# CatOfTheCannals/MPI_blockchain

Measured on AMD Instinct MI355X. Metric: SHA-256 nonce trials/sec (whole job) + % int32 VALU peak, higher is better.
Workload: dtype u32

## Files before the change

mpi_blockchain_amd/csrc/pow_api.cpp:

```cpp
#include <sys/prctl.h>

#include <algorithm>
#include <chrono>
#include <cstdio>
#include <cstring>
#include <ctime>
#include <thread>
#include <vector>

#include "pow_ctx.h"

#ifndef POW_WAIT_POLL_US
#define POW_WAIT_POLL_US 50
#endif

const pow_test_hooks* pow_hooks = nullptr;

namespace {

int stage_result(pow_ctx* ctx, bool with_tail, uint64_t abs_start);

void fill_watch(const pow_ctx* ctx, PowWatch& w, uint64_t abs_start) {
  memset(&w, 0, sizeof w);
  w.watch_epoch = ctx->watch_epoch && ctx->armed.load(std::memory_order_acquire) ? 1u : 0u;
  w.host_epoch = ctx->d_epoch;
  w.launch_epoch = ctx->launch_epoch;
  w.abs_start = abs_start;
  if (ctx->board && !ctx->board_off) {
    w.board = ctx->board_dev;
    w.board_mine = const_cast<unsigned long long*>(ctx->board_dev) + ctx->board_slot;
    w.board_n = (uint32_t)pow_board_nslots(ctx->board);
    w.board_tag = ctx->board_tag;
  }
}

uint64_t board_peer_min(const pow_ctx* ctx) {
  uint64_t m = UINT64_MAX;
  if (ctx->board && !ctx->board_off) pow_board_peek(ctx->board, ctx->board_slot, ctx->board_tag, &m);
  return m;
}

int set_dev(const pow_ctx* ctx) {
  HIP_OK(hipSetDevice(ctx->device));
  return POW_OK;
}

int stream_wait(pow_ctx* ctx, const char* what, uint64_t t0, uint64_t deadline_ns, bool nap) {
  HIP_OK(hipEventRecord(ctx->ev_block, ctx->stream));
  const int slack = nap ? prctl(PR_GET_TIMERSLACK, 0, 0, 0, 0) : 0;
  if (slack > 1000) prctl(PR_SET_TIMERSLACK, 1000ul, 0, 0, 0);
  hipError_t q;
  bool late = false;
  for (uint32_t n = 1; (q = hipEventQuery(ctx->ev_block)) == hipErrorNotReady; ++n) {
    if (nap) std::this_thread::sleep_for(std::chrono::microseconds(POW_WAIT_POLL_US));
    if ((nap || (n & 255u) == 0) && mono_ns() > deadline_ns) {
      late = true;
      break;
    }
  }
  if (slack > 1000) prctl(PR_SET_TIMERSLACK, (unsigned long)slack, 0, 0, 0);
  if (late) {
    ctx->wedged = true;
    return fail(POW_EHIP, "%s: watchdog: not complete after %.3f s (deadline %.3f s; hipStreamQuery: %s); "
                "the context must not be reused",
                what, (mono_ns() - t0) * 1e-9, (deadline_ns - t0) * 1e-9, hipGetErrorString(hipStreamQuery(ctx->stream)));
  }
  HIP_OK(q);
  HIP_OK(hipStreamSynchronize(ctx->stream));
  return POW_OK;
}

int stream_wait_for(pow_ctx* ctx, const char* what, uint64_t extra_ns) {
  const uint64_t t0 = mono_ns();
  return stream_wait(ctx, what, t0, t0 + ctx->watchdog_ns + extra_ns, false);
}

unsigned grid_for(const pow_ctx* ctx, uint32_t n_prefix) {
  const uint64_t want = ((uint64_t)n_prefix + 255) / 256;
  return (unsigned)std::max<uint64_t>(1, std::min<uint64_t>(want, ctx->grid_full));
}

int run_search(pow_ctx* ctx, uint64_t start, uint64_t count, unsigned diff, uint32_t mode,
               uint32_t* dev_out, uint32_t cap) {
  PowLaunch L;
  int rc = make_launch(start, count, diff, cap, mode, &L);
  if (rc) return rc;
  if (ctx->sentinel_idle && mode >= 1) L.mode |= POW_LAUNCH_SENTINEL_IDLE;
  if (int rc2 = stage_result(ctx, true, start)) return rc2;
  const unsigned grid = grid_for(ctx, L.n_prefix);
  if (pow_hooks)
    if (int rc2 = pow_hooks->before_launch(ctx)) return rc2;
  HIP_OK(hipEventRecord(ctx->ev0, ctx->stream));
  HIP_OK(pow_launch_search((int)mode, diff > 32 || ctx->force_full, grid, ctx->stream, ctx->d_consts, L, dev_out,
                           ctx->d_res));
  HIP_OK(hipEventRecord(ctx->ev1, ctx->stream));
  HIP_OK(hipMemcpyAsync(ctx->h_res, ctx->d_res, sizeof(PowResult), hipMemcpyDeviceToHost, ctx->stream));
  {
    char what[160];
    snprintf(what, sizeof what, "search kernel (mode %u, %llu counters from %llu, d = %u)", mode,
             (unsigned long long)count, (unsigned long long)start, diff);
    const uint64_t t0 = mono_ns();
    if (int rc2 = stream_wait(ctx, what, t0, t0 + ctx->watchdog_ns + 2ull * count, count >= (1ull << 26)))
      return rc2;
  }
  float ms = 0;
  HIP_OK(hipEventElapsedTime(&ms, ctx->ev0, ctx->ev1));
  ctx->stats.kernel_ms += ms;
  ctx->stats.launches += 1;
  ctx->stats.hashes += mode >= 1 ? ctx->h_res->hashes : (uint64_t)L.n_prefix * POW_J;
  return POW_OK;
}

int wait_published(pow_ctx* ctx, const volatile uint32_t* done, const volatile uint32_t* started, uint32_t seq,
                   const char* what, uint64_t t0, uint64_t deadline_ns) {
  for (uint32_t n = 1; __atomic_load_n(const_cast<const uint32_t*>(done), __ATOMIC_ACQUIRE) != seq; ++n) {
    if ((n & 0xFFFFu) != 0) continue;
    int st;
    hipError_t q = hipSuccess;
    if (ctx->aql) {
      st = pow_hooks->path_status(ctx);
    } else {
      q = hipStreamQuery(ctx->stream);
      st = q == hipErrorNotReady ? 1 : q == hipSuccess ? 0 : -1;
    }
    if (st == 1) {
      if (mono_ns() <= deadline_ns) continue;
      const uint32_t seen = __atomic_load_n(const_cast<const uint32_t*>(done), __ATOMIC_ACQUIRE);
      if (seen == seq) break;
      std::string path = "launch path hip, hipStreamQuery: not ready";
      if (ctx->aql) path = pow_hooks->path_diag(ctx);
      const uint32_t st_word = __atomic_load_n(const_cast<const uint32_t*>(started), __ATOMIC_ACQUIRE);
      ctx->wedged = true;
      return fail(POW_EHIP,
                  "%s: watchdog: no result after %.3f s (seq %u, done word %u; the kernel %s (started word %u); %s); "
                  "the context must not be reused",
                  what, (mono_ns() - t0) * 1e-9, seq, seen,
                  st_word == seq ? "started: its first workgroup ran" : "never started", st_word, path.c_str());
    }
    if (__atomic_load_n(const_cast<const uint32_t*>(done), __ATOMIC_ACQUIRE) == seq) break;
    if (st < 0 && ctx->aql) return fail(POW_EHIP, "%s: the dispatch queue reported HSA status 0x%x", what, -st);
    HIP_OK(q);
    return fail(POW_EHIP, "%s ended without publishing its result (seq %u, done word %u)", what, seq,
                __atomic_load_n(const_cast<const uint32_t*>(done), __ATOMIC_ACQUIRE));
  }
  return POW_OK;
}

}

int launch_hash_one(pow_ctx* ctx, const PowMsg& M, uint32_t seq, uint64_t deadline_ns) {
  if (pow_hooks) {
    if (int sent = pow_hooks->dispatch_hash_one(ctx, M, seq, deadline_ns)) return sent < 0 ? sent : POW_OK;
    if (int rc = pow_hooks->before_launch(ctx)) return rc;
  }
  HIP_OK(pow_launch_hash_one(ctx->stream, M, ctx->d_one, seq));
  return POW_OK;
}

int launch_search_lat(pow_ctx* ctx, bool full, bool any, bool asm_groups, unsigned grid, const PowLaunchLat& L,
                      uint64_t deadline_ns) {
  if (pow_hooks) {
    if (int sent = pow_hooks->dispatch_lat(ctx, full, any, asm_groups, grid, L, deadline_ns))
      return sent < 0 ? sent : POW_OK;
// ... 22 lines not shown
  if (int rc = wait_published(ctx, &ctx->h_lat->done, &ctx->h_lat->started, L.seq, "latency kernel", t0, deadline))
    return rc;
  memcpy(ctx->h_res, (const void*)ctx->h_lat, sizeof(PowResult));
  const double ms = (double)ctx->h_res->ticks / ctx->realtime_khz;
  ctx->stats.kernel_ms += ms;
  ctx->stats.launches += 1;
  ctx->stats.hashes += ctx->h_res->hashes;
  return POW_OK;
}

int upload_consts(pow_ctx* ctx, const pow_block* tmpl) {
  pow_build_consts(tmpl, &ctx->h_blob->consts);
  const PowConsts& C = ctx->h_blob->consts;
  PowConstsLat& Q = ctx->lat_consts;
  memcpy(Q.kw, C.kw, sizeof Q.kw);
  memcpy(Q.st0, C.st0, sizeof Q.st0);
  memcpy(Q.kw0, C.kw0, sizeof Q.kw0);
  memcpy(Q.k, C.k, sizeof Q.k);
  memcpy(Q.w0raw, C.w0raw, sizeof Q.w0raw);
  ctx->consts_dirty = true;
  return POW_OK;
}

int stage_result(pow_ctx* ctx, bool with_tail, uint64_t abs_start) {
  PowResult& r = ctx->h_blob->res;
  memset(&r, 0, sizeof r);
  r.min_rel = ~0ull;
  r.peer_abs = ~0ull;
  fill_watch(ctx, r.watch, abs_start);
  if (with_tail) {
    r.tail_buf = ctx->d_tail;
    r.tail_cap = ctx->tail_cap;
  }
  const size_t off = ctx->consts_dirty ? 0 : offsetof(PowBlob, res);
  HIP_OK(hipMemcpyAsync((char*)ctx->d_blob + off, (const char*)ctx->h_blob + off, sizeof(PowBlob) - off,
                        hipMemcpyHostToDevice, ctx->stream));
  ctx->consts_dirty = false;
  return POW_OK;
}

}

bool cancel_moved(const volatile uint32_t* cancel_word, uint32_t epoch) {
  return cancel_word && __atomic_load_n(const_cast<const uint32_t*>(cancel_word), __ATOMIC_ACQUIRE) != epoch;
}

int pow_ctx_device(const pow_ctx* ctx) { return ctx->device; }
bool pow_ctx_wedged(const pow_ctx* ctx) { return ctx->wedged; }
void pow_ctx_set_stats(pow_ctx* ctx, const pow_stats& s) { ctx->stats = s; }
void* pow_ctx_stream(const pow_ctx* ctx) { return (void*)ctx->stream; }
int pow_ctx_stream_wait(pow_ctx* ctx, const char* what, uint64_t budget_ns) {
  return stream_wait_for(ctx, what, budget_ns);
}

extern "C" {

int pow_device_count(int* n) {
  if (!n) return fail(POW_EINVAL, "null");
  *n = 0;
  HIP_OK(hipGetDeviceCount(n));
// ... 17 lines not shown
  ctx->cu_count = prop.multiProcessorCount;
  {
    int rt = 0;
    if (hipDeviceGetAttribute(&rt, hipDeviceAttributeWallClockRate, device) == hipSuccess && rt > 0)
      ctx->realtime_khz = rt;
  }
  ctx->clock_khz = prop.clockRate;
  snprintf(ctx->name, sizeof ctx->name, "%s", prop.name);
  ctx->grid_full = (unsigned)prop.multiProcessorCount * 8u - 1u;
  if (pow_hooks) pow_hooks->configure(ctx);
  int rc = POW_OK;
  auto chk = [&](hipError_t e, const char* what) {
    if (e != hipSuccess && rc == POW_OK) rc = fail(POW_EHIP, "%s: %s", what, hipGetErrorString(e));
  };
  chk(hipStreamCreateWithFlags(&ctx->stream, hipStreamNonBlocking), "hipStreamCreate");
  chk(hipEventCreate(&ctx->ev0), "hipEventCreate");
  chk(hipEventCreate(&ctx->ev1), "hipEventCreate");
  chk(hipEventCreateWithFlags(&ctx->ev_block, hipEventDisableTiming), "hipEventCreate");
  chk(hipMalloc(&ctx->d_blob, sizeof(PowBlob)), "hipMalloc consts/result");
  if (ctx->d_blob) chk(hipMemsetAsync(ctx->d_blob, 0, sizeof(PowBlob), ctx->stream), "hipMemsetAsync");
  chk(hipMalloc(&ctx->d_lat, sizeof(PowResult)), "hipMalloc latency result");
  chk(hipHostMalloc(&ctx->h_lat, sizeof(PowResult), hipHostMallocMapped | hipHostMallocCoherent),
      "hipHostMalloc latency result");
  if (ctx->d_lat && ctx->h_lat) {
    PowResult* init = ctx->h_lat;
    memset(init, 0, sizeof *init);
    init->min_rel = ~0ull;
    init->peer_abs = ~0ull;
    chk(hipMemcpyAsync(ctx->d_lat, init, sizeof *init, hipMemcpyHostToDevice, ctx->stream), "hipMemcpyAsync");
    if (rc == POW_OK) rc = stream_wait_for(ctx, "pow_init copies", 0);
    chk(hipHostGetDevicePointer((void**)&ctx->d_lat_host, ctx->h_lat, 0), "hipHostGetDevicePointer");
  }
  chk(hipHostMalloc(&ctx->h_one, sizeof(PowHashOut), hipHostMallocMapped | hipHostMallocCoherent),
      "hipHostMalloc hash result");
  if (ctx->h_one) {
    memset(ctx->h_one, 0, sizeof(PowHashOut));
    chk(hipHostGetDevicePointer((void**)&ctx->d_one, ctx->h_one, 0), "hipHostGetDevicePointer");
  }
  chk(hipHostMalloc(&ctx->h_epoch, 64, hipHostMallocMapped | hipHostMallocCoherent), "hipHostMalloc epoch");
  if (ctx->h_epoch) {
    *ctx->h_epoch = 0;
    chk(hipHostGetDevicePointer((void**)&ctx->d_epoch, ctx->h_epoch, 0), "hipHostGetDevicePointer");
  }
  chk(hipHostMalloc(&ctx->h_blob, sizeof(PowBlob), hipHostMallocDefault), "hipHostMalloc staging");
  if (ctx->d_blob) {
    ctx->d_consts = &ctx->d_blob->consts;
    ctx->d_res = &ctx->d_blob->res;
  }
  chk(hipHostMalloc(&ctx->h_res, sizeof(PowResult), hipHostMallocDefault), "hipHostMalloc");
  ctx->tail_cap = ctx->grid_full * 4u * 32u;
  chk(hipMalloc(&ctx->d_tail, (size_t)ctx->tail_cap * sizeof(uint32_t)), "hipMalloc sweep tail");
  if (rc == POW_OK && pow_hooks) pow_hooks->open_path(ctx);
// ... 32 lines not shown
  if (ctx->h_brec) (void)hipHostFree(ctx->h_brec);
  (void)hipFree(ctx->d_race);
  (void)hipFree(ctx->d_rin);
  (void)hipFree(ctx->d_rslot);
  if (ctx->h_race) (void)hipHostFree(ctx->h_race);
  if (ctx->h_rin) (void)hipHostFree(ctx->h_rin);
  if (ctx->h_res) (void)hipHostFree(ctx->h_res);
  if (ctx->ev0) (void)hipEventDestroy(ctx->ev0);
  if (ctx->ev1) (void)hipEventDestroy(ctx->ev1);
  if (ctx->ev_block) (void)hipEventDestroy(ctx->ev_block);
  if (ctx->stream) (void)hipStreamDestroy(ctx->stream);
  if (ctx->h_epoch) (void)hipHostFree(ctx->h_epoch);
  (void)hipFree(ctx->d_lat);
  if (ctx->h_lat) (void)hipHostFree(ctx->h_lat);
  if (ctx->h_one) (void)hipHostFree(ctx->h_one);
  delete ctx;
}

int pow_warmup(pow_ctx* ctx) {
  if (!ctx) return fail(POW_EINVAL, "null");
  if (int rc = set_dev(ctx)) return rc;
  PowLaunch L;
  memset(&L, 0, sizeof L);
  PowLaunchLat LL;
  memset(&LL, 0, sizeof LL);
  LL.nwg = 1;
  for (int mode = 0; mode < 3; ++mode)
    for (int full = 0; full < 2; ++full)
      HIP_OK(pow_launch_search(mode, full != 0, 1, ctx->stream, ctx->d_consts, L, nullptr, ctx->d_res));
  for (int any = 0; any < 2; ++any)
    for (int full = 0; full < 2; ++full)
      for (int grp = 0; grp < 2; ++grp)
        HIP_OK(pow_launch_search_lat(full != 0, any != 0, grp != 0, 1, ctx->stream, ctx->lat_consts, LL,
                                     ctx->d_lat, ctx->d_lat_host));
  HIP_OK(pow_launch_hash(0, ctx->stream, nullptr, nullptr));
  PowMsg M;
  memset(&M, 0, sizeof M);
  HIP_OK(pow_launch_hash_one(ctx->stream, M, ctx->d_one, 0));
  if (int rc = stream_wait_for(ctx, "warm-up launches", 0)) return rc;
  if (pow_hooks)
    if (int rc = pow_hooks->warm_path(ctx, LL, M)) return rc;
  pow_block b;
  memset(&b, 0, sizeof b);
  return pow_hash_blocks(ctx, &b, 1, nullptr, nullptr);
}

// ... 225 lines not shown
  uint64_t step = use_lat ? std::max<uint64_t>(1ull << 12, 1ull << (dcap + 4))
                          : (any ? 1ull << 30 : std::max<uint64_t>(1ull << 12, 1ull << std::min(dcap + 2, 30u)));
  auto preempted = [&](uint64_t next) {
    const uint64_t m = board_peer_min(ctx);
    return any ? m != UINT64_MAX : m < next;
  };
  uint64_t done = 0;
  bool first = true;
  while (done < ctr_count) {
    if (cancel_moved(cancel_word, epoch) || preempted(ctr_start + done)) break;
    const bool lat = first && use_lat;
    const uint64_t cap = lat ? ctx->lat_max : (uint64_t)1 << 30;
    const uint64_t n = std::min<uint64_t>(std::min<uint64_t>(step, cap), ctr_count - done);
    const uint64_t s0 = ctr_start + done;
    if (int rc = lat ? run_search_lat(ctx, s0, n, diff_bits, any, lat_wps)
                     : run_search(ctx, s0, n, diff_bits, any ? 2 : 1, nullptr, 0))
      return rc;
    first = false;
    done += n;
    if (cancel_moved(cancel_word, epoch) || ctx->h_res->cancelled) break;
    if (ctx->h_res->min_rel != ~0ull) {
      const PowResult& r = *ctx->h_res;
      const PowHit* h = nullptr;
      for (uint32_t k = 0; lat && k < std::min<uint32_t>(r.nhit, POW_HITS); ++k) {
        const PowHit* c = &r.hit[k];
        if (any ? (!h || c->rel < h->rel) : c->rel == r.min_rel) h = c;
      }
      const uint64_t ctr = s0 + (h ? h->rel : r.min_rel);
      if (!any && board_peer_min(ctx) < ctr) break;
      *out = *tmpl;
      pow_nonce_from_counter(ctr, out->nonce);
      char hx[65];
      if (h) {
        digest_out(h->digest, nullptr, hx);
      } else {
        const pow_stats keep = ctx->stats;
        ctx->watch_epoch = false;
        ctx->board_off = true;
        const int rc = run_search_lat(ctx, ctr, 1, 0, true, 1);
        ctx->board_off = false;
        if (rc) return rc;
        ctx->stats = keep;
        const PowResult& w = *ctx->h_res;
        if (w.nhit < 1 || w.hit[0].rel != 0) return fail(POW_EHIP, "winner re-hash recorded no digest");
        digest_out(w.hit[0].digest, nullptr, hx);
      }
      memcpy(out->block_hash, hx, 65);
// ... 504 lines not shown
```

mpi_blockchain_amd/csrc/pow_kernels.hip:

```cpp
#include <hip/hip_runtime.h>
#include <stdint.h>

#include "pow_template.h"
#include "sha256_dev.h"

using namespace powdev;


namespace {

__device__ __forceinline__ uint32_t digit_char(uint32_t d) {
  return d + (d < 26u ? 97u : (d < 52u ? 39u : 0xFFFFFFFCu));
}

__device__ __forceinline__ unsigned long long uniform64(unsigned long long v) {
  uint32_t lo = __builtin_amdgcn_readfirstlane((uint32_t)v);
  uint32_t hi = __builtin_amdgcn_readfirstlane((uint32_t)(v >> 32));
  return ((unsigned long long)hi << 32) | lo;
}

typedef const __attribute__((address_space(4))) uint32_t* cptr;

__device__ __forceinline__ cptr as_const(const uint32_t* p) {
  return (cptr)(const __attribute__((address_space(1))) uint32_t*)p;
}

__device__ __forceinline__ cptr pin(cptr p, uint32_t dep) {
  asm volatile("" : "+s"(p) : "v"(dep));
  return p;
}

template <bool ASM>
__device__ __forceinline__ void const_chunk_lds(St& t, const uint32_t* lkw) {
  if (ASM) {
    POW_SB();
    const uint4 v0 = *reinterpret_cast<const uint4*>(lkw);
    POW_SB();
    t = rounds4_asm_from(t, v0.x, v0.y, v0.z, v0.w);
#pragma unroll
    for (int g = 4; g < 64; g += 4) {
      POW_SB();
      const uint4 v = *reinterpret_cast<const uint4*>(lkw + g);
      POW_SB();
      rounds4_asm(t, v.x, v.y, v.z, v.w);
    }
    POW_SB();
  } else {
#pragma unroll
    for (int g = 0; g < 64; g += 4) {
      const uint4 v = *reinterpret_cast<const uint4*>(lkw + g);
      round_kw_o(t, v.x);
      round_kw_o(t, v.y);
// ... 52 lines not shown
  const uint32_t n = nst & ~31u;
  unsigned long long got = 0;
  if (lane == 0) got = atomicAdd(&res->count, (unsigned long long)n);
  const unsigned long long base = uniform64(got);
  const uint32_t i = lane * 4u;
  if (i < n) {
    const uint32_t e0 = wst[i], e1 = wst[i + 1u], e2 = wst[i + 2u], e3 = wst[i + 3u];
    const unsigned long long o = base + i;
    if (o + 4u <= cap && ((uintptr_t)out & 15u) == 0) {
      *reinterpret_cast<uint4*>(out + o) = make_uint4(e0, e1, e2, e3);
    } else {
      if (o < cap) out[o] = e0;
      if (o + 1u < cap) out[o + 1u] = e1;
      if (o + 2u < cap) out[o + 2u] = e2;
      if (o + 3u < cap) out[o + 3u] = e3;
    }
  }
  const uint32_t rem = nst - n;
  const uint32_t t = lane < rem ? wst[n + lane] : 0u;
  if (lane < rem) wst[lane] = t;
  nst = rem;
}

__device__ __forceinline__ void flush_tail(const uint32_t* wst, uint32_t nst, uint32_t lane, PowResult* res) {
  uint32_t got = 0;
  if (lane == 0) got = atomicAdd(&res->tail, nst);
  const uint32_t base = __builtin_amdgcn_readfirstlane(got);
  uint32_t* const tail = res->tail_buf;
  const uint32_t tail_cap = res->tail_cap;
  if (lane < nst && base + lane < tail_cap) tail[base + lane] = wst[lane];
}

__device__ __forceinline__ bool poll_stop(const PowWatch& w, unsigned int* cancelled, unsigned long long* peer_abs,
                                          unsigned long long lowest_abs) {
  const uint32_t watch = w.watch_epoch;
  const unsigned long long* const board = w.board;
  if (!watch && !board) return false;
  if (blockIdx.x == 0 && threadIdx.x < 64u) {
    const uint32_t lane = threadIdx.x;
    if (watch) {
      const unsigned int now = __hip_atomic_load(w.host_epoch, __ATOMIC_RELAXED, __HIP_MEMORY_SCOPE_SYSTEM);
      if ((uint32_t)__builtin_amdgcn_readfirstlane(now) != w.launch_epoch && lane == 0)
        __hip_atomic_store(cancelled, 1u, __ATOMIC_RELAXED, __HIP_MEMORY_SCOPE_AGENT);
    }
    if (board) {
      unsigned long long c = ~0ull;
      if (lane < w.board_n && board + lane != w.board_mine) {
        const unsigned long long v = __hip_atomic_load(board + lane, __ATOMIC_RELAXED, __HIP_MEMORY_SCOPE_SYSTEM);
        if ((uint32_t)(v >> POW_BOARD_SHIFT) == w.board_tag && (v & POW_BOARD_NONE) != POW_BOARD_NONE)
          c = v & POW_BOARD_NONE;
      }
#pragma unroll
// ... 15 lines not shown
  if (mine)
    __hip_atomic_store(mine, ((unsigned long long)w.board_tag << POW_BOARD_SHIFT) | (w.abs_start + rel),
                       __ATOMIC_RELAXED, __HIP_MEMORY_SCOPE_SYSTEM);
}

__device__ __forceinline__ bool full_test(const uint32_t H[8], uint32_t d) { return leading_zero_bits(H) >= d; }

}

#define POW_BATCH 8u

template <int MODE, bool FULL>
__global__ __launch_bounds__(256) __attribute__((amdgpu_num_sgpr(80), amdgpu_waves_per_eu(8))) void pow_search(
    const PowConsts* __restrict__ C, PowLaunch L, uint32_t* __restrict__ out,
    PowResult* __restrict__ res) {
  const uint32_t lane = threadIdx.x & 63u;
  uint32_t iters = 0;
  __shared__ __attribute__((aligned(16))) uint32_t stage[4][256];
  uint32_t* wst = stage[threadIdx.x >> 6];
  uint32_t nst = 0;
  uint32_t mymin = 0xFFFFFFFFu;
  __shared__ __attribute__((aligned(16))) uint32_t lkw[4 * 64];
  lkw[threadIdx.x] = (&C->kw[0][0])[threadIdx.x];
  __shared__ uint32_t sibs_done;
  __shared__ uint32_t wg_tick;
  __shared__ unsigned long long wg_ring[4];
  __shared__ uint32_t wg_reads[4];
  if (threadIdx.x == 0) {
    sibs_done = 0;
    wg_tick = 0;
  }
  if (threadIdx.x < 4) {
    wg_ring[threadIdx.x] = 0;
    wg_reads[threadIdx.x] = POW_BATCH - 1u;
  }
  __syncthreads();

  const bool sentinel_idle = MODE >= 1 && (L.mode & POW_LAUNCH_SENTINEL_IDLE) && blockIdx.x == 0 && threadIdx.x < 64u;
  for (;;) {
    if (sentinel_idle) break;
    uint32_t got = 0;
    if (lane == 0) {
      const uint32_t t = atomicAdd(&wg_tick, 1u);
      const uint32_t b = t / POW_BATCH, slot = t % POW_BATCH;
      unsigned long long* const ring = &wg_ring[b & 3u];
      uint32_t* const reads = &wg_reads[b & 3u];
      if (slot == 0) {
        got = atomicAdd(&res->next, 64u * POW_BATCH);
        while (__hip_atomic_load(reads, __ATOMIC_ACQUIRE, __HIP_MEMORY_SCOPE_WORKGROUP) != POW_BATCH - 1u)
          __builtin_amdgcn_s_sleep(1);
        __hip_atomic_store(reads, 0u, __ATOMIC_RELAXED, __HIP_MEMORY_SCOPE_WORKGROUP);
        __hip_atomic_store(ring, ((unsigned long long)(b + 1u) << 32) | got, __ATOMIC_RELEASE,
                           __HIP_MEMORY_SCOPE_WORKGROUP);
      } else {
        unsigned long long v;
        while ((uint32_t)((v = __hip_atomic_load(ring, __ATOMIC_ACQUIRE, __HIP_MEMORY_SCOPE_WORKGROUP)) >> 32) !=
               b + 1u)
          __builtin_amdgcn_s_sleep(1);
        got = (uint32_t)v + 64u * slot;
        __hip_atomic_fetch_add(reads, 1u, __ATOMIC_RELEASE, __HIP_MEMORY_SCOPE_WORKGROUP);
      }
    }
    const uint32_t rbase = __builtin_amdgcn_readfirstlane(got);
    if (rbase >= L.n_prefix) break;
    if (MODE >= 1) {
      unsigned long long f =
          __hip_atomic_load(&res->min_rel, __ATOMIC_RELAXED, __HIP_MEMORY_SCOPE_AGENT);
      f = uniform64(f);
      long long lo = (long long)rbase * 62 - (long long)L.off0;
      if (MODE == 2 && f != ~0ull) break;
      if (lo > 0 && f < (unsigned long long)lo) break;
      if (poll_stop(res->watch, &res->cancelled, &res->peer_abs,
                    MODE == 2 ? ~0ull : res->watch.abs_start + (lo > 0 ? (unsigned long long)lo : 0ull)))
        break;
    }
    const uint32_t r = rbase + lane;

    uint32_t dg[8];
    {
      uint32_t x = r, carry = 0;
#pragma unroll
      for (int i = 7; i >= 0; --i) {
        uint32_t q = x / 62u;
        uint32_t s = L.base_digit[i] + (x - q * 62u) + carry;
        x = q;
        carry = s >= 62u ? 1u : 0u;
        dg[i] = carry ? s - 62u : s;
      }
    }
    const uint32_t W1 = (digit_char(dg[0]) << 24) | (digit_char(dg[1]) << 16) |
                        (digit_char(dg[2]) << 8) | digit_char(dg[3]);
    const uint32_t W2 = (digit_char(dg[4]) << 24) | (digit_char(dg[5]) << 16) |
                        (digit_char(dg[6]) << 8) | digit_char(dg[7]);

    St s2{C->st0[0], C->st0[1], C->st0[2], C->st0[3], C->st0[4], C->st0[5], C->st0[6], C->st0[7]};
    round_k_w(s2, K[1], W1);
    round_k_w(s2, K[2], W2);
    const uint32_t W16 = C->u16 + ssig0(W1);
    const uint32_t W17 = C->u17 + ssig0(W2) + W1;
    const uint32_t c18 = ssig1(W16) + W2;
    const uint32_t c19 = ssig1(W17) + C->u19;
    const uint32_t c23 = W16 + C->u23;
    const uint32_t c24 = W17 + C->u24;
    const uint32_t c31 = ssig0(W16) + C->w15;
    const uint32_t c32 = ssig0(W17) + W16;
    const uint32_t P3 = s2.h + bsig1(s2.e) + ch(s2.e, s2.f, s2.g);
    const uint32_t A3 = P3 + bsig0(s2.a) + maj(s2.a, s2.b, s2.c);
    const uint32_t E3 = s2.d + P3;

    bool stop = false;
    for (uint32_t j = 0; j < POW_J; ++j) {
      if (MODE == 1 && j != 0 && (j & 1u) == 0) {
        unsigned long long f =
            __hip_atomic_load(&res->min_rel, __ATOMIC_RELAXED, __HIP_MEMORY_SCOPE_AGENT);
        f = uniform64(f);
        long long lo = (long long)rbase * 62 + j - (long long)L.off0;
        if (lo > 0 && f < (unsigned long long)lo) break;
        if (poll_stop(res->watch, &res->cancelled, &res->peer_abs,
                      res->watch.abs_start + (lo > 0 ? (unsigned long long)lo : 0ull))) {
          stop = true;
          break;
        }
      }
      if (MODE == 2 && j != 0) {
        unsigned long long f =
            __hip_atomic_load(&res->min_rel, __ATOMIC_RELAXED, __HIP_MEMORY_SCOPE_AGENT);
        if (uniform64(f) != ~0ull || poll_stop(res->watch, &res->cancelled, &res->peer_abs, ~0ull)) {
          stop = true;
          break;
        }
      }
      ++iters;
      cptr Cb = as_const(reinterpret_cast<const uint32_t*>(C));
      cptr J = pin(Cb, s2.a ^ j);
      const uint32_t kw3 = J[PC_KW3 + j];
      const St s4{A3 + kw3, s2.a, s2.b, s2.c, E3 + kw3, s2.e, s2.f, s2.g};
      asm volatile(".p2align 3");
      POW_SB();
      St s = rounds4_kws_asm_from(s4, J[PC_KW0 + 4], J[PC_KW0 + 5], J[PC_KW0 + 6], J[PC_KW0 + 7]);
#pragma unroll
      for (int i = 8; i < 16; i += 4) {
        POW_SB();
        rounds4_kws_asm(s, J[PC_KW0 + i], J[PC_KW0 + i + 1], J[PC_KW0 + i + 2], J[PC_KW0 + i + 3]);
      }
      uint32_t w[64];
      w[16] = W16;
      w[17] = W17;
      auto rnd4 = [&](int i, cptr Kx) {
        if (i >= 36) {
          POW_SB();
// ... 32 lines not shown
        cptr K3 = pin(Cb + PC_K, s.e);
#pragma unroll
        for (int i = 48; i < 64; i += 4) rnd4(i, K3);
      }
      uint32_t H[8] = {IV[0] + s.a, IV[1] + s.b, IV[2] + s.c, IV[3] + s.d,
                       IV[4] + s.e, IV[5] + s.f, IV[6] + s.g, IV[7] + s.h};

      St Hs{H[0], H[1], H[2], H[3], H[4], H[5], H[6], H[7]};
      St t = Hs;
      const_chunk_lds<true>(t, lkw);
#pragma unroll
      for (int c = 1; c < 4; ++c) const_chunk_lds_ff(Hs, t, lkw + 64 * c);
      const uint32_t h0 = Hs.a + t.a;

      bool hit = h0 <= L.thr;
      if (FULL && hit) {
        uint32_t D[8] = {h0, Hs.b + t.b, Hs.c + t.c, Hs.d + t.d,
                         Hs.e + t.e, Hs.f + t.f, Hs.g + t.g, Hs.h + t.h};
        hit = full_test(D, L.diff);
      }
      if (MODE != 0) {
        if (__builtin_expect(hit, 0)) {
          const unsigned long long rel = (unsigned long long)r * 62ull + j - L.off0;
          if (rel < L.count && rel < atomicMin(&res->min_rel, rel)) publish_hit(res->watch, rel);
        }
      } else {
        bool ok = false;
        uint32_t relv = 0;
        if (__builtin_expect(hit, 0)) {
          const unsigned long long rel = (unsigned long long)r * 62ull + j - L.off0;
          ok = rel < L.count;
          relv = (uint32_t)rel;
          if (ok && relv < mymin) mymin = relv;
          if (ok && relv == 0xFFFFFFFFu) atomicMin(&res->min_rel, rel);
        }
        const unsigned long long m = __ballot(ok);
        if (m) {
          const uint32_t rank = __builtin_amdgcn_mbcnt_hi((uint32_t)(m >> 32),
                                                          __builtin_amdgcn_mbcnt_lo((uint32_t)m, 0u));
          if (ok) wst[nst + rank] = relv;
          nst += (uint32_t)__popcll(m);
          if (nst >= 192) flush_stage(wst, nst, lane, res, out, L.cap);
        }
      }
    }
    if (MODE >= 1 && stop) break;
  }
  if (MODE == 0) {
    if (nst >= 32) flush_stage(wst, nst, lane, res, out, L.cap);
    if (nst) flush_tail(wst, nst, lane, res);
#pragma unroll
    for (int off = 32; off > 0; off >>= 1) {
      const uint32_t o = __shfl_xor(mymin, off, 64);
      mymin = o < mymin ? o : mymin;
    }
    if (lane == 0 && mymin != 0xFFFFFFFFu) atomicMin(&res->min_rel, (unsigned long long)mymin);
  }
  if (MODE >= 1) {
    if (blockIdx.x == 0) {
      if (threadIdx.x >= 64u) {
        if (lane == 0) __hip_atomic_fetch_add(&sibs_done, 1u, __ATOMIC_RELAXED, __HIP_MEMORY_SCOPE_WORKGROUP);
      } else if (res->watch.watch_epoch || res->watch.board) {
        for (;;) {
          const uint32_t sd = __hip_atomic_load(&sibs_done, __ATOMIC_RELAXED, __HIP_MEMORY_SCOPE_WORKGROUP);
          const uint32_t ex = __hip_atomic_load(&res->wg_exits, __ATOMIC_RELAXED, __HIP_MEMORY_SCOPE_AGENT);
          if (__builtin_amdgcn_readfirstlane(sd) >= (blockDim.x >> 6) - 1u &&
              __builtin_amdgcn_readfirstlane(ex) >= gridDim.x - 1u)
            break;
          (void)poll_stop(res->watch, &res->cancelled, &res->peer_abs, ~0ull);
          __builtin_amdgcn_s_sleep(32);
        }
      }
    }
    __shared__ uint32_t wave_iters[4];
    if ((threadIdx.x & 63u) == 0) wave_iters[threadIdx.x >> 6] = iters;
    __syncthreads();
    if (threadIdx.x == 0) {
      atomicAdd(&res->hashes,
                (unsigned long long)(wave_iters[0] + wave_iters[1] + wave_iters[2] + wave_iters[3]) * 64ull);
      if (blockIdx.x != 0) atomicAdd(&res->wg_exits, 1u);
    }
  }
}

template __global__ void pow_search<0, false>(const PowConsts*, PowLaunch, uint32_t*, PowResult*);
template __global__ void pow_search<0, true>(const PowConsts*, PowLaunch, uint32_t*, PowResult*);
template __global__ void pow_search<1, false>(const PowConsts*, PowLaunch, uint32_t*, PowResult*);
template __global__ void pow_search<1, true>(const PowConsts*, PowLaunch, uint32_t*, PowResult*);
template __global__ void pow_search<2, false>(const PowConsts*, PowLaunch, uint32_t*, PowResult*);
template __global__ void pow_search<2, true>(const PowConsts*, PowLaunch, uint32_t*, PowResult*);

template <bool FULL, bool ANY, bool ASM>
__global__ __launch_bounds__(256) void pow_search_lat(
    const PowConstsLat C0, PowLaunchLat L, PowResult* __restrict__ res, PowResult* __restrict__ hout) {
  (void)C0;
  const cptr Cb = (cptr)__builtin_amdgcn_kernarg_segment_ptr();
  const uint32_t lane = threadIdx.x & 63u;
  const uint32_t wave = __builtin_amdgcn_readfirstlane(blockIdx.x * 4u + (threadIdx.x >> 6));
  const uint32_t nwaves = L.nwg * 4u;
  uint32_t iters = 0;
  bool wrote_hit = false;
  __shared__ uint32_t wg_iters;
  if (threadIdx.x == 0) wg_iters = 0;
// ... 232 lines not shown
```

mpi_blockchain_amd/csrc/pow_template.h:

```cpp
#pragma once
#include <stdint.h>

#define POW_J 62

struct PowConsts {
  uint32_t kw[4][64];
  uint32_t st0[8];
  uint32_t kw0[16];
  uint32_t w0, w1_unused, w2_unused, w3lo;
  uint32_t u16;
  uint32_t u17;
  uint32_t u19;
  uint32_t u20, u21, u22;
  uint32_t u23, u24;
  uint32_t u25[6];
  uint32_t w15;
  uint32_t pad[3];
  uint32_t kw3[POW_J];
  uint32_t u18[POW_J];
  uint32_t w3[POW_J];
  uint32_t k[64];
  uint32_t w0raw[16];
};

// ... 24 lines not shown

struct PowWatch {
  const unsigned int* host_epoch;
  const unsigned long long* board;
  unsigned long long* board_mine;
  unsigned long long abs_start;
  uint32_t watch_epoch;
  uint32_t launch_epoch;
  uint32_t board_n;
  uint32_t board_tag;
};

struct PowLaunchLat {
  uint32_t base_digit[9];
  uint32_t thr;
  uint32_t diff;
  uint32_t seq;
  uint64_t count;
  PowWatch watch;
  uint32_t nwg;
  uint32_t pad;
};

struct PowLaunch {
  uint32_t base_digit[8];
  uint32_t n_prefix;
  uint32_t off0;
  uint64_t count;
  uint32_t thr;
  uint32_t diff;
  uint32_t cap;
  uint32_t mode;
};
#define POW_LAUNCH_SENTINEL_IDLE 0x100u

#define POW_HITS 8
struct PowHit {
  unsigned long long rel;
  uint32_t digest[8];
};

struct PowResult {
  unsigned long long min_rel;
  unsigned long long hashes;
  unsigned long long count;
  unsigned int next;
  unsigned int wg_exits;
  unsigned int tail;
  unsigned int tail_cap;
  unsigned int* tail_buf;
  unsigned int nhit;
  unsigned int cancelled;
  unsigned long long peer_abs;
  PowWatch watch;
  unsigned long long t_start;
  unsigned long long ticks;
  unsigned int done;
  unsigned int started;
  PowHit hit[POW_HITS];
};

struct PowMsg {
  uint32_t kw[5][64];
};
struct PowHashOut {
  uint32_t digest[8];
  unsigned long long ticks;
  unsigned int done;
  unsigned int started;
};

struct PowBlob {
  PowConsts consts;
  alignas(256) PowResult res;
};

#ifdef __cplusplus
// ... 19 lines not shown
```

Baseline: 9.138 billion.

## Publish search results via mapped host memory and self-reset device state in kernel

Per-launch watch and tail parameters now travel in kernel arguments, so the host-to-device copy that staged the result struct before every launch is gone. The last workgroup to finish resets the device result struct and writes the summary, hits and a done sequence word into mapped coherent host memory. The host polls that word instead of recording events and issuing a device-to-host copy. Kernel time is taken from device realtime ticks except in mode 0. This adds last-block election logic, more kernel-argument reads in the hot loop and extra atomics on hits, and correctness now depends on the in-kernel reset.

```diff
diff --git a/mpi_blockchain_amd/csrc/pow_api.cpp b/mpi_blockchain_amd/csrc/pow_api.cpp
--- a/mpi_blockchain_amd/csrc/pow_api.cpp
+++ b/mpi_blockchain_amd/csrc/pow_api.cpp
@@ -17,8 +17,6 @@
 const pow_test_hooks* pow_hooks = nullptr;
 
 namespace {
-
-int stage_result(pow_ctx* ctx, bool with_tail, uint64_t abs_start);
 
 void fill_watch(const pow_ctx* ctx, PowWatch& w, uint64_t abs_start) {
   memset(&w, 0, sizeof w);
@@ -45,20 +43,16 @@
   return POW_OK;
 }
 
-int stream_wait(pow_ctx* ctx, const char* what, uint64_t t0, uint64_t deadline_ns, bool nap) {
+int stream_wait(pow_ctx* ctx, const char* what, uint64_t t0, uint64_t deadline_ns) {
   HIP_OK(hipEventRecord(ctx->ev_block, ctx->stream));
-  const int slack = nap ? prctl(PR_GET_TIMERSLACK, 0, 0, 0, 0) : 0;
-  if (slack > 1000) prctl(PR_SET_TIMERSLACK, 1000ul, 0, 0, 0);
   hipError_t q;
   bool late = false;
   for (uint32_t n = 1; (q = hipEventQuery(ctx->ev_block)) == hipErrorNotReady; ++n) {
-    if (nap) std::this_thread::sleep_for(std::chrono::microseconds(POW_WAIT_POLL_US));
-    if ((nap || (n & 255u) == 0) && mono_ns() > deadline_ns) {
+    if ((n & 255u) == 0 && mono_ns() > deadline_ns) {
       late = true;
       break;
     }
   }
-  if (slack > 1000) prctl(PR_SET_TIMERSLACK, (unsigned long)slack, 0, 0, 0);
   if (late) {
     ctx->wedged = true;
     return fail(POW_EHIP, "%s: watchdog: not complete after %.3f s (deadline %.3f s; hipStreamQuery: %s); "
@@ -72,7 +66,7 @@
 
 int stream_wait_for(pow_ctx* ctx, const char* what, uint64_t extra_ns) {
   const uint64_t t0 = mono_ns();
-  return stream_wait(ctx, what, t0, t0 + ctx->watchdog_ns + extra_ns, false);
+  return stream_wait(ctx, what, t0, t0 + ctx->watchdog_ns + extra_ns);
 }
 
 unsigned grid_for(const pow_ctx* ctx, uint32_t n_prefix) {
@@ -80,44 +74,34 @@
   return (unsigned)std::max<uint64_t>(1, std::min<uint64_t>(want, ctx->grid_full));
 }
 
-int run_search(pow_ctx* ctx, uint64_t start, uint64_t count, unsigned diff, uint32_t mode,
-               uint32_t* dev_out, uint32_t cap) {
-  PowLaunch L;
-  int rc = make_launch(start, count, diff, cap, mode, &L);
-  if (rc) return rc;
-  if (ctx->sentinel_idle && mode >= 1) L.mode |= POW_LAUNCH_SENTINEL_IDLE;
-  if (int rc2 = stage_result(ctx, true, start)) return rc2;
-  const unsigned grid = grid_for(ctx, L.n_prefix);
-  if (pow_hooks)
-    if (int rc2 = pow_hooks->before_launch(ctx)) return rc2;
-  HIP_OK(hipEventRecord(ctx->ev0, ctx->stream));
-  HIP_OK(pow_launch_search((int)mode, diff > 32 || ctx->force_full, grid, ctx->stream, ctx->d_consts, L, dev_out,
-                           ctx->d_res));
-  HIP_OK(hipEventRecord(ctx->ev1, ctx->stream));
-  HIP_OK(hipMemcpyAsync(ctx->h_res, ctx->d_res, sizeof(PowResult), hipMemcpyDeviceToHost, ctx->stream));
-  {
-    char what[160];
-    snprintf(what, sizeof what, "search kernel (mode %u, %llu counters from %llu, d = %u)", mode,
-             (unsigned long long)count, (unsigned long long)start, diff);
-    const uint64_t t0 = mono_ns();
-    if (int rc2 = stream_wait(ctx, what, t0, t0 + ctx->watchdog_ns + 2ull * count, count >= (1ull << 26)))
-      return rc2;
-  }
-  float ms = 0;
-  HIP_OK(hipEventElapsedTime(&ms, ctx->ev0, ctx->ev1));
-  ctx->stats.kernel_ms += ms;
-  ctx->stats.launches += 1;
-  ctx->stats.hashes += mode >= 1 ? ctx->h_res->hashes : (uint64_t)L.n_prefix * POW_J;
-  return POW_OK;
-}
-
 int wait_published(pow_ctx* ctx, const volatile uint32_t* done, const volatile uint32_t* started, uint32_t seq,
-                   const char* what, uint64_t t0, uint64_t deadline_ns) {
+                   const char* what, uint64_t t0, uint64_t deadline_ns, uint64_t nap_from_ns = UINT64_MAX,
+                   const char* late = "watchdog: no result after", bool on_stream = false) {
+  const bool direct = ctx->aql && !on_stream;
+  struct Slack {
+    int was = 0;
+    void lower() {
+      if (was) return;
+      was = prctl(PR_GET_TIMERSLACK, 0, 0, 0, 0);
+      if (was > 1000) prctl(PR_SET_TIMERSLACK, 1000ul, 0, 0, 0);
+    }
+    ~Slack() {
+      if (was > 1000) prctl(PR_SET_TIMERSLACK, (unsigned long)was, 0, 0, 0);
+    }
+  } slack;
+  bool nap = nap_from_ns == 0;
   for (uint32_t n = 1; __atomic_load_n(const_cast<const uint32_t*>(done), __ATOMIC_ACQUIRE) != seq; ++n) {
-    if ((n & 0xFFFFu) != 0) continue;
+    if (nap) {
+      slack.lower();
+      std::this_thread::sleep_for(std::chrono::microseconds(POW_WAIT_POLL_US));
+      if ((n & 15u) != 0) continue;
+    } else {
+      if (nap_from_ns != UINT64_MAX && (n & 0xFFu) == 0 && mono_ns() >= nap_from_ns) nap = true;
+      if ((n & 0xFFFFu) != 0) continue;
+    }
     int st;
     hipError_t q = hipSuccess;
-    if (ctx->aql) {
+    if (direct) {
       st = pow_hooks->path_status(ctx);
     } else {
       q = hipStreamQuery(ctx->stream);
@@ -128,17 +112,17 @@
       const uint32_t seen = __atomic_load_n(const_cast<const uint32_t*>(done), __ATOMIC_ACQUIRE);
       if (seen == seq) break;
       std::string path = "launch path hip, hipStreamQuery: not ready";
-      if (ctx->aql) path = pow_hooks->path_diag(ctx);
+      if (direct) path = pow_hooks->path_diag(ctx);
       const uint32_t st_word = __atomic_load_n(const_cast<const uint32_t*>(started), __ATOMIC_ACQUIRE);
       ctx->wedged = true;
       return fail(POW_EHIP,
-                  "%s: watchdog: no result after %.3f s (seq %u, done word %u; the kernel %s (started word %u); %s); "
+                  "%s: %s %.3f s (seq %u, done word %u; the kernel %s (started word %u); %s); "
                   "the context must not be reused",
-                  what, (mono_ns() - t0) * 1e-9, seq, seen,
+                  what, late, (mono_ns() - t0) * 1e-9, seq, seen,
                   st_word == seq ? "started: its first workgroup ran" : "never started", st_word, path.c_str());
     }
     if (__atomic_load_n(const_cast<const uint32_t*>(done), __ATOMIC_ACQUIRE) == seq) break;
-    if (st < 0 && ctx->aql) return fail(POW_EHIP, "%s: the dispatch queue reported HSA status 0x%x", what, -st);
+    if (st < 0 && direct) return fail(POW_EHIP, "%s: the dispatch queue reported HSA status 0x%x", what, -st);
     HIP_OK(q);
     return fail(POW_EHIP, "%s ended without publishing its result (seq %u, done word %u)", what, seq,
                 __atomic_load_n(const_cast<const uint32_t*>(done), __ATOMIC_ACQUIRE));
@@ -207,20 +191,50 @@
   return POW_OK;
 }
 
-int stage_result(pow_ctx* ctx, bool with_tail, uint64_t abs_start) {
-  PowResult& r = ctx->h_blob->res;
-  memset(&r, 0, sizeof r);
-  r.min_rel = ~0ull;
-  r.peer_abs = ~0ull;
-  fill_watch(ctx, r.watch, abs_start);
-  if (with_tail) {
-    r.tail_buf = ctx->d_tail;
-    r.tail_cap = ctx->tail_cap;
-  }
-  const size_t off = ctx->consts_dirty ? 0 : offsetof(PowBlob, res);
-  HIP_OK(hipMemcpyAsync((char*)ctx->d_blob + off, (const char*)ctx->h_blob + off, sizeof(PowBlob) - off,
-                        hipMemcpyHostToDevice, ctx->stream));
-  ctx->consts_dirty = false;
+int run_search(pow_ctx* ctx, uint64_t start, uint64_t count, unsigned diff, uint32_t mode,
+               uint32_t* dev_out, uint32_t cap) {
+  PowLaunch L;
+  int rc = make_launch(start, count, diff, cap, mode, &L);
+  if (rc) return rc;
+  if (ctx->sentinel_idle && mode >= 1) L.mode |= POW_LAUNCH_SENTINEL_IDLE;
+  fill_watch(ctx, L.watch, start);
+  L.tail_buf = ctx->d_tail;
+  L.tail_cap = ctx->tail_cap;
+  L.hout = ctx->d_lat_host;
+  const unsigned grid = grid_for(ctx, L.n_prefix);
+  L.nwg = grid;
+  if (++ctx->lat_seq == 0) ctx->lat_seq = 1;
+  L.seq = ctx->lat_seq;
+  if (ctx->consts_dirty) {
+    HIP_OK(hipMemcpyAsync(ctx->d_consts, &ctx->h_blob->consts, sizeof(PowConsts), hipMemcpyHostToDevice,
+                          ctx->stream));
+    ctx->consts_dirty = false;
+  }
+  if (pow_hooks)
+    if (int rc2 = pow_hooks->before_launch(ctx)) return rc2;
+  if (mode == 0) HIP_OK(hipEventRecord(ctx->ev0, ctx->stream));
+  HIP_OK(pow_launch_search((int)mode, diff > 32 || ctx->force_full, grid, ctx->stream, ctx->d_consts, L, dev_out,
+                           ctx->d_res));
+  if (mode == 0) HIP_OK(hipEventRecord(ctx->ev1, ctx->stream));
+  char what[160];
+  snprintf(what, sizeof what, "search kernel (mode %u, %llu counters from %llu, d = %u)", mode,
+           (unsigned long long)count, (unsigned long long)start, diff);
+  const uint64_t t0 = mono_ns(), deadline = t0 + ctx->watchdog_ns + 2ull * count;
+  const uint64_t expect = mode == 0 || diff >= 32 ? count : std::min<uint64_t>(count, 1ull << diff);
+  if (int rc2 = wait_published(ctx, &ctx->h_lat->done, &ctx->h_lat->started, L.seq, what, t0, deadline,
+                               expect >= (1ull << 26) ? 0 : t0 + 8000000ull, "watchdog: not complete after", true))
+    return rc2;
+  memcpy(ctx->h_res, (const void*)ctx->h_lat, sizeof(PowResult));
+  double ms = (double)ctx->h_res->ticks / ctx->realtime_khz;
+  if (mode == 0) {
+    if (int rc2 = stream_wait(ctx, what, t0, deadline)) return rc2;
+    float ev_ms = 0;
+    HIP_OK(hipEventElapsedTime(&ev_ms, ctx->ev0, ctx->ev1));
+    ms = ev_ms;
+  }
+  ctx->stats.kernel_ms += ms;
+  ctx->stats.launches += 1;
+  ctx->stats.hashes += mode >= 1 ? ctx->h_res->hashes : (uint64_t)L.n_prefix * POW_J;
   return POW_OK;
 }
 
@@ -284,12 +298,13 @@
   chk(hipMalloc(&ctx->d_lat, sizeof(PowResult)), "hipMalloc latency result");
   chk(hipHostMalloc(&ctx->h_lat, sizeof(PowResult), hipHostMallocMapped | hipHostMallocCoherent),
       "hipHostMalloc latency result");
-  if (ctx->d_lat && ctx->h_lat) {
+  if (ctx->d_blob && ctx->d_lat && ctx->h_lat) {
     PowResult* init = ctx->h_lat;
     memset(init, 0, sizeof *init);
     init->min_rel = ~0ull;
     init->peer_abs = ~0ull;
     chk(hipMemcpyAsync(ctx->d_lat, init, sizeof *init, hipMemcpyHostToDevice, ctx->stream), "hipMemcpyAsync");
+    chk(hipMemcpyAsync(&ctx->d_blob->res, init, sizeof *init, hipMemcpyHostToDevice, ctx->stream), "hipMemcpyAsync");
     if (rc == POW_OK) rc = stream_wait_for(ctx, "pow_init copies", 0);
     chk(hipHostGetDevicePointer((void**)&ctx->d_lat_host, ctx->h_lat, 0), "hipHostGetDevicePointer");
   }
@@ -368,6 +383,8 @@
   if (int rc = set_dev(ctx)) return rc;
   PowLaunch L;
   memset(&L, 0, sizeof L);
+  L.nwg = 1;
+  L.hout = ctx->d_lat_host;
   PowLaunchLat LL;
   memset(&LL, 0, sizeof LL);
   LL.nwg = 1;
@@ -639,7 +656,7 @@
     if (ctx->h_res->min_rel != ~0ull) {
       const PowResult& r = *ctx->h_res;
       const PowHit* h = nullptr;
-      for (uint32_t k = 0; lat && k < std::min<uint32_t>(r.nhit, POW_HITS); ++k) {
+      for (uint32_t k = 0; k < std::min<uint32_t>(r.nhit, POW_HITS); ++k) {
         const PowHit* c = &r.hit[k];
         if (any ? (!h || c->rel < h->rel) : c->rel == r.min_rel) h = c;
       }
diff --git a/mpi_blockchain_amd/csrc/pow_kernels.hip b/mpi_blockchain_amd/csrc/pow_kernels.hip
--- a/mpi_blockchain_amd/csrc/pow_kernels.hip
+++ b/mpi_blockchain_amd/csrc/pow_kernels.hip
@@ -28,6 +28,14 @@
 __device__ __forceinline__ cptr pin(cptr p, uint32_t dep) {
   asm volatile("" : "+s"(p) : "v"(dep));
   return p;
+}
+
+static_assert(alignof(PowLaunch) == 8, "PowLaunch follows K1's first (pointer) argument");
+__device__ __forceinline__ const PowLaunch& launch_args_here() {
+  const __attribute__((address_space(4))) char* ka =
+      (const __attribute__((address_space(4))) char*)__builtin_amdgcn_kernarg_segment_ptr();
+  asm volatile("" : "+s"(ka));
+  return *(const PowLaunch*)(const char*)(ka + 8);
 }
 
 template <bool ASM>
@@ -126,12 +134,11 @@
   nst = rem;
 }
 
-__device__ __forceinline__ void flush_tail(const uint32_t* wst, uint32_t nst, uint32_t lane, PowResult* res) {
+__device__ __forceinline__ void flush_tail(const uint32_t* wst, uint32_t nst, uint32_t lane, PowResult* res,
+                                           uint32_t* tail, uint32_t tail_cap) {
   uint32_t got = 0;
   if (lane == 0) got = atomicAdd(&res->tail, nst);
   const uint32_t base = __builtin_amdgcn_readfirstlane(got);
-  uint32_t* const tail = res->tail_buf;
-  const uint32_t tail_cap = res->tail_cap;
   if (lane < nst && base + lane < tail_cap) tail[base + lane] = wst[lane];
 }
 
@@ -193,17 +200,24 @@
   uint32_t mymin = 0xFFFFFFFFu;
   __shared__ __attribute__((aligned(16))) uint32_t lkw[4 * 64];
   lkw[threadIdx.x] = (&C->kw[0][0])[threadIdx.x];
-  __shared__ uint32_t sibs_done;
+  __shared__ uint32_t waves_out;
+  __shared__ uint32_t wg_iters;
   __shared__ uint32_t wg_tick;
   __shared__ unsigned long long wg_ring[4];
   __shared__ uint32_t wg_reads[4];
   if (threadIdx.x == 0) {
-    sibs_done = 0;
+    waves_out = 0;
+    wg_iters = 0;
     wg_tick = 0;
   }
   if (threadIdx.x < 4) {
     wg_ring[threadIdx.x] = 0;
     wg_reads[threadIdx.x] = POW_BATCH - 1u;
+  }
+  if (blockIdx.x == 0 && threadIdx.x == 0) {
+    __hip_atomic_store(&res->t_start, __builtin_amdgcn_s_memrealtime(), __ATOMIC_RELAXED, __HIP_MEMORY_SCOPE_AGENT);
+    const PowLaunch& A = launch_args_here();
+    __hip_atomic_store(&A.hout->started, A.seq, __ATOMIC_RELAXED, __HIP_MEMORY_SCOPE_SYSTEM);
   }
   __syncthreads();
 
@@ -241,8 +255,9 @@
       long long lo = (long long)rbase * 62 - (long long)L.off0;
       if (MODE == 2 && f != ~0ull) break;
       if (lo > 0 && f < (unsigned long long)lo) break;
-      if (poll_stop(res->watch, &res->cancelled, &res->peer_abs,
-                    MODE == 2 ? ~0ull : res->watch.abs_start + (lo > 0 ? (unsigned long long)lo : 0ull)))
+      const PowWatch& W = launch_args_here().watch;
+      if (poll_stop(W, &res->cancelled, &res->peer_abs,
+                    MODE == 2 ? ~0ull : W.abs_start + (lo > 0 ? (unsigned long long)lo : 0ull)))
         break;
     }
     const uint32_t r = rbase + lane;
@@ -287,8 +302,8 @@
         f = uniform64(f);
         long long lo = (long long)rbase * 62 + j - (long long)L.off0;
         if (lo > 0 && f < (unsigned long long)lo) break;
-        if (poll_stop(res->watch, &res->cancelled, &res->peer_abs,
-                      res->watch.abs_start + (lo > 0 ? (unsigned long long)lo : 0ull))) {
+        const PowWatch& W = launch_args_here().watch;
+        if (poll_stop(W, &res->cancelled, &res->peer_abs, W.abs_start + (lo > 0 ? (unsigned long long)lo : 0ull))) {
           stop = true;
           break;
         }
@@ -296,7 +311,7 @@
       if (MODE == 2 && j != 0) {
         unsigned long long f =
             __hip_atomic_load(&res->min_rel, __ATOMIC_RELAXED, __HIP_MEMORY_SCOPE_AGENT);
-        if (uniform64(f) != ~0ull || poll_stop(res->watch, &res->cancelled, &res->peer_abs, ~0ull)) {
+        if (uniform64(f) != ~0ull || poll_stop(launch_args_here().watch, &res->cancelled, &res->peer_abs, ~0ull)) {
           stop = true;
           break;
         }
@@ -375,7 +390,21 @@
       if (MODE != 0) {
         if (__builtin_expect(hit, 0)) {
           const unsigned long long rel = (unsigned long long)r * 62ull + j - L.off0;
-          if (rel < L.count && rel < atomicMin(&res->min_rel, rel)) publish_hit(res->watch, rel);
+          if (rel < L.count && rel < atomicMin(&res->min_rel, rel)) {
+            publish_hit(launch_args_here().watch, rel);
+            const uint32_t slot = atomicAdd(&res->nhit, 1u);
+            if (slot < POW_HITS) {
+              PowHit* const rec = &res->hit[slot];
+              const uint32_t D[8] = {h0, Hs.b + t.b, Hs.c + t.c, Hs.d + t.d,
+                                     Hs.e + t.e, Hs.f + t.f, Hs.g + t.g, Hs.h + t.h};
+              __hip_atomic_store(&rec->rel, rel, __ATOMIC_RELAXED, __HIP_MEMORY_SCOPE_AGENT);
+#pragma unroll
+              for (int k = 0; k < 8; ++k)
+                __hip_atomic_store(&rec->digest[k], D[k], __ATOMIC_RELAXED, __HIP_MEMORY_SCOPE_AGENT);
+            }
+            __builtin_amdgcn_fence(__ATOMIC_RELEASE, "agent");
+            asm volatile("s_waitcnt vmcnt(0)" ::: "memory");
+          }
         }
       } else {
         bool ok = false;
@@ -401,7 +430,10 @@
   }
   if (MODE == 0) {
     if (nst >= 32) flush_stage(wst, nst, lane, res, out, L.cap);
-    if (nst) flush_tail(wst, nst, lane, res);
+    if (nst) {
+      const PowLaunch& A = launch_args_here();
+      flush_tail(wst, nst, lane, res, A.tail_buf, A.tail_cap);
+    }
 #pragma unroll
     for (int off = 32; off > 0; off >>= 1) {
       const uint32_t o = __shfl_xor(mymin, off, 64);
@@ -409,29 +441,70 @@
     }
     if (lane == 0 && mymin != 0xFFFFFFFFu) atomicMin(&res->min_rel, (unsigned long long)mymin);
   }
+  const uint32_t xlane = __builtin_amdgcn_mbcnt_hi(~0u, __builtin_amdgcn_mbcnt_lo(~0u, 0u));
   if (MODE >= 1) {
-    if (blockIdx.x == 0) {
-      if (threadIdx.x >= 64u) {
-        if (lane == 0) __hip_atomic_fetch_add(&sibs_done, 1u, __ATOMIC_RELAXED, __HIP_MEMORY_SCOPE_WORKGROUP);
-      } else if (res->watch.watch_epoch || res->watch.board) {
+    if (blockIdx.x == 0 && threadIdx.x < 64u) {
+      const PowLaunch& A = launch_args_here();
+      if (A.watch.watch_epoch || A.watch.board) {
         for (;;) {
-          const uint32_t sd = __hip_atomic_load(&sibs_done, __ATOMIC_RELAXED, __HIP_MEMORY_SCOPE_WORKGROUP);
-          const uint32_t ex = __hip_atomic_load(&res->wg_exits, __ATOMIC_RELAXED, __HIP_MEMORY_SCOPE_AGENT);
-          if (__builtin_amdgcn_readfirstlane(sd) >= (blockDim.x >> 6) - 1u &&
-              __builtin_amdgcn_readfirstlane(ex) >= gridDim.x - 1u)
-            break;
-          (void)poll_stop(res->watch, &res->cancelled, &res->peer_abs, ~0ull);
+          const uint32_t sd = __hip_atomic_load(&waves_out, __ATOMIC_RELAXED, __HIP_MEMORY_SCOPE_WORKGROUP);
+          const uint32_t ex =
+              (uint32_t)__hip_atomic_load(&res->hashes, __ATOMIC_RELAXED, __HIP_MEMORY_SCOPE_AGENT);
+          if (__builtin_amdgcn_readfirstlane(sd) >= 3u && __builtin_amdgcn_readfirstlane(ex) >= A.nwg - 1u) break;
+          (void)poll_stop(launch_args_here().watch, &res->cancelled, &res->peer_abs, ~0ull);
           __builtin_amdgcn_s_sleep(32);
         }
       }
     }
-    __shared__ uint32_t wave_iters[4];
-    if ((threadIdx.x & 63u) == 0) wave_iters[threadIdx.x >> 6] = iters;
-    __syncthreads();
-    if (threadIdx.x == 0) {
-      atomicAdd(&res->hashes,
-                (unsigned long long)(wave_iters[0] + wave_iters[1] + wave_iters[2] + wave_iters[3]) * 64ull);
-      if (blockIdx.x != 0) atomicAdd(&res->wg_exits, 1u);
+  }
+  asm volatile("s_waitcnt vmcnt(0)" ::: "memory");
+  uint32_t ticket = 0;
+  if (xlane == 0) {
+    if (MODE >= 1) __hip_atomic_fetch_add(&wg_iters, iters, __ATOMIC_RELAXED, __HIP_MEMORY_SCOPE_WORKGROUP);
+    ticket = __hip_atomic_fetch_add(&waves_out, 1u, __ATOMIC_ACQ_REL, __HIP_MEMORY_SCOPE_WORKGROUP);
+  }
+  if (__builtin_amdgcn_readfirstlane(ticket) == 3u) {
+    const PowLaunch& A = launch_args_here();
+    const unsigned long long mine =
+        MODE >= 1 ? (unsigned long long)__builtin_amdgcn_readfirstlane(
+                        __hip_atomic_load(&wg_iters, __ATOMIC_RELAXED, __HIP_MEMORY_SCOPE_WORKGROUP))
+                  : 0ull;
+    unsigned long long old = 0;
+    if (xlane == 0)
+      old = __hip_atomic_fetch_add(&res->hashes, (mine << 32) | 1ull, __ATOMIC_RELAXED, __HIP_MEMORY_SCOPE_AGENT);
+    old = uniform64(old);
+    if ((uint32_t)old == A.nwg - 1u) {
+      __builtin_amdgcn_fence(__ATOMIC_ACQUIRE, "agent");
+      PowResult* const hout = A.hout;
+      const uint32_t nhit = __hip_atomic_load(&res->nhit, __ATOMIC_RELAXED, __HIP_MEMORY_SCOPE_AGENT);
+      if (MODE >= 1 && xlane < (nhit < POW_HITS ? nhit : POW_HITS)) {
+        hout->hit[xlane].rel = __hip_atomic_load(&res->hit[xlane].rel, __ATOMIC_RELAXED, __HIP_MEMORY_SCOPE_AGENT);
+#pragma unroll
+        for (int k = 0; k < 8; ++k)
+          hout->hit[xlane].digest[k] =
+              __hip_atomic_load(&res->hit[xlane].digest[k], __ATOMIC_RELAXED, __HIP_MEMORY_SCOPE_AGENT);
+      }
+      if (xlane == 0) {
+        hout->min_rel = __hip_atomic_load(&res->min_rel, __ATOMIC_RELAXED, __HIP_MEMORY_SCOPE_AGENT);
+        hout->hashes = ((old >> 32) + mine) * 64ull;
+        hout->count = __hip_atomic_load(&res->count, __ATOMIC_RELAXED, __HIP_MEMORY_SCOPE_AGENT);
+        hout->tail = __hip_atomic_load(&res->tail, __ATOMIC_RELAXED, __HIP_MEMORY_SCOPE_AGENT);
+        hout->nhit = nhit;
+        hout->cancelled = __hip_atomic_load(&res->cancelled, __ATOMIC_RELAXED, __HIP_MEMORY_SCOPE_AGENT);
+        hout->ticks = __builtin_amdgcn_s_memrealtime() -
+                      __hip_atomic_load(&res->t_start, __ATOMIC_RELAXED, __HIP_MEMORY_SCOPE_AGENT);
+        res->min_rel = ~0ull;
+        res->hashes = 0;
+        res->count = 0;
+        res->next = 0;
+        res->tail = 0;
+        res->nhit = 0;
+        res->cancelled = 0;
+        res->peer_abs = ~0ull;
+      }
+      __builtin_amdgcn_fence(__ATOMIC_RELEASE, "");
+      asm volatile("s_waitcnt vmcnt(0)" ::: "memory");
+      if (xlane == 0) __hip_atomic_store(&hout->done, A.seq, __ATOMIC_RELAXED, __HIP_MEMORY_SCOPE_SYSTEM);
     }
   }
 }
diff --git a/mpi_blockchain_amd/csrc/pow_template.h b/mpi_blockchain_amd/csrc/pow_template.h
--- a/mpi_blockchain_amd/csrc/pow_template.h
+++ b/mpi_blockchain_amd/csrc/pow_template.h
@@ -70,6 +70,7 @@
   uint32_t pad;
 };
 
+struct PowResult;
 struct PowLaunch {
   uint32_t base_digit[8];
   uint32_t n_prefix;
@@ -79,6 +80,13 @@
   uint32_t diff;
   uint32_t cap;
   uint32_t mode;
+  PowWatch watch;
+  uint32_t* tail_buf;
+  uint32_t tail_cap;
+  uint32_t seq;
+  PowResult* hout;
+  uint32_t nwg;
+  uint32_t pad;
 };
 #define POW_LAUNCH_SENTINEL_IDLE 0x100u
 
@@ -95,12 +103,10 @@
   unsigned int next;
   unsigned int wg_exits;
   unsigned int tail;
-  unsigned int tail_cap;
-  unsigned int* tail_buf;
   unsigned int nhit;
   unsigned int cancelled;
+  unsigned int pad;
   unsigned long long peer_abs;
-  PowWatch watch;
   unsigned long long t_start;
   unsigned long long ticks;
   unsigned int done;
```

After: 9.134 billion. No clear change (-0.0%).
